# skywoodsz/qm_control

Hardware: NVIDIA H100
Metric: mpc_wbc_iters_per_s (higher is better)
Workload: dtype f64

## Files before the change

### qm_control_b200/csrc/capi.cu

```cuda
#include <cuda_runtime.h>

#include <algorithm>
#include <cmath>
#include <cstdio>
#include <cstring>
#include <string>
#include <vector>

#include "../../include/qmb200.h"
#include "host/qm_config.h"
#include "kernels/mpc_api.cuh"
#include "kernels/ctrl_api.cuh"
#include "kernels/sim_api.cuh"
#include "kernels/payload_est_api.cuh"
#include "kernels/state_est_api.cuh"
#include "kernels/attitude_api.cuh"
#include "kernels/slip_api.cuh"
#include "kernels/gait_api.cuh"

namespace qmb {
void launch_wbc_update(const DevModel* mdl, int B, const double* x_des, const double* u_des, const double* rbd, const int32_t* mode, const double* period, const double* time,
                       double* input_last, int variant, double* cmd, int32_t* status, cudaStream_t stream, int b0 = 0, int b1 = -1, int32_t* diag = nullptr,
                       const double* srbd = nullptr, const double* payload = nullptr);
int wbc_configure_device();
int mpc_configure_device();
}

using namespace qmb;

static thread_local std::string g_create_error;

struct RobotArray {
  int width; std::vector<double> host; double* d = nullptr;
  const double* dev() const { return host.empty() ? nullptr : d; }
};

struct qmb200_handle {
  HostModel hm;
  DevModel* d_model = nullptr;
  int B = 0, nmax = 0, variant = 0, device = 0;
  cudaStream_t stream = nullptr;
  std::string err, task_file, reference_file;
  int64_t launches = 0;
  double *d_xdes = nullptr, *d_udes = nullptr, *d_input_last = nullptr;
  int32_t *d_mode = nullptr, *d_wbc_diag = nullptr, *d_safety = nullptr;
  char* stage = nullptr; size_t stage_bytes = 0;
  MpcBuffers mpc;
  std::vector<void*> allocs;
  bool profiling = false; cudaEvent_t ev[8] = {nullptr};
  double kernel_ms[7] = {0, 0, 0, 0, 0, 0, 0}; int64_t kernel_calls = 0; bool ev_pending = false;
  static constexpr int MAX_CHUNKS = 8;
  TargetParams target_prm{}; ControlLawParams law_prm{0, 0.0, 0.5};
  double hw_delay = 0.0; double *hw_ring_cmd = nullptr, *hw_ring_stamp = nullptr; int32_t* hw_ring_state = nullptr;
  void* comm = nullptr; int comm_ranks = 0, comm_rank = 0; double* d_send = nullptr;
  SimParams sim_prm{};
  RobotArray mu{1}, payload{8};
  RobotArray terrain{3};
  struct { std::vector<double> host; double* d = nullptr; int n_tiles = 0, nx = 0, ny = 0; double cell = 0.0; } tiles;
  RobotArray mpayload{8}, srbd{SRBD_DBL};
  qmb200_payload_est_params est_prm{}; double* d_est = nullptr;
  qmb200_sensor_params sensor_prm{};
  qmb200_state_est_params se_prm{}; double* d_se = nullptr;
  RobotArray se_ground{3};
  qmb200_attitude_params at_prm{}; double* d_at = nullptr;
  qmb200_slip_params sl_prm{}; double* d_sl = nullptr;
  struct {
    std::vector<GsTemplate> table; GsTemplate* d_table = nullptr; GsRobot* d_robots = nullptr; int32_t* d_cursor = nullptr;
    double* d_t = nullptr; int32_t* d_tmpl = nullptr; double* d_vel = nullptr; int n_cmd = 0; double stance_time = 0.0;
    int32_t* d_ee_kind = nullptr; double* d_ee = nullptr;
  } gs;
  bool model_on_device = false;
  int chunks = 1; cudaStream_t cs[MAX_CHUNKS] = {nullptr}; cudaEvent_t fork_ev = nullptr, join_ev[MAX_CHUNKS] = {nullptr};
};

namespace {
template <class T> bool dalloc(qmb200_handle* h, T** p, size_t count) {
  void* q = nullptr; cudaError_t e = cudaMalloc(&q, count * sizeof(T));
  if (e != cudaSuccess) { h->err = std::string("cudaMalloc failed: ") + cudaGetErrorString(e); return false; }
  cudaMemsetAsync(q, 0, count * sizeof(T), h->stream); h->allocs.push_back(q); *p = static_cast<T*>(q); return true;
}
SimParams default_sim_params();
qmb200_payload_est_params default_est_params();
qmb200_state_est_params default_state_est_params(const DevModel& d);
qmb200_attitude_params default_attitude_params();
qmb200_slip_params default_slip_params();
int fail(qmb200_handle* h, const std::string& msg) { if (h) h->err = msg; else g_create_error = msg; return -1; }
#define QMB_CUDA(h, call) do { cudaError_t e_ = (call); if (e_ != cudaSuccess) return fail(h, std::string(#call) + ": " + cudaGetErrorString(e_)); } while (0)

HostModel config_model(const qmb200_config* cfg) {
  HostModel hm = build_host_model(cfg->task_file, cfg->urdf_file, cfg->reference_file, cfg->wbc_gains_file ? cfg->wbc_gains_file : "");
  if (cfg->time_horizon > 0) hm.dev.time_horizon = cfg->time_horizon;
  if (cfg->dt > 0) hm.dev.dt = cfg->dt;
  return hm;
}
int push_model(qmb200_handle* h) {
  QMB_CUDA(h, cudaMemcpyAsync(h->d_model, &h->hm.dev, sizeof(DevModel), cudaMemcpyHostToDevice, h->stream)); QMB_CUDA(h, cudaStreamSynchronize(h->stream)); return 0;
}

struct RobotRows { RobotArray* a; const double* rows; };
int set_robot_arrays(qmb200_handle* h, std::initializer_list<RobotRows> sets) {
  const size_t B = (size_t)h->B;
  QMB_CUDA(h, cudaSetDevice(h->device));
  for (const RobotRows& s : sets) if (s.rows && !s.a->d && !dalloc(h, &s.a->d, B * s.a->width)) return -4;
  QMB_CUDA(h, cudaDeviceSynchronize());
  for (const RobotRows& s : sets) if (s.rows) QMB_CUDA(h, cudaMemcpy(s.a->d, s.rows, B * s.a->width * 8, cudaMemcpyHostToDevice));
  for (const RobotRows& s : sets) { if (s.rows) s.a->host.assign(s.rows, s.rows + B * s.a->width); else s.a->host.clear(); }
  return 0;
}

class Staging {
 public:
  static constexpr size_t ROBOT_BYTES = 243 * 8, ALIGN = 256, STAGE_SLICES = 10;
  explicit Staging(qmb200_handle* h) : h_(h) {}
  int open() {
    QMB_CUDA(h_, cudaSetDevice(h_->device));
    if (!h_->stage) {
      const size_t bytes = (size_t)h_->B * ROBOT_BYTES + STAGE_SLICES * ALIGN;
      if (!dalloc(h_, &h_->stage, bytes)) return -4;
      h_->stage_bytes = bytes;
    }
    return 0;
  }
  template <class T> const T* in(const T* src, size_t n) {
    if (!src) return nullptr;
    T* d = slice<T>(n); note(cudaMemcpyAsync(d, src, n * sizeof(T), cudaMemcpyHostToDevice, h_->stream)); return d;
  }
  template <class T> T* inout(T* p, size_t n) { T* d = const_cast<T*>(in<T>(p, n)); back_.push_back({p, d, n * sizeof(T)}); return d; }
  template <class T> T* out(T* p, size_t n) { T* d = slice<T>(n); back_.push_back({p, d, n * sizeof(T)}); return d; }
  int done(int rc) {
    if (rc) return rc;
    for (const Back& b : back_) note(cudaMemcpyAsync(b.host, b.dev, b.bytes, cudaMemcpyDeviceToHost, h_->stream));
    note(cudaStreamSynchronize(h_->stream));
    return err_.empty() ? 0 : fail(h_, err_);
  }

 private:
  struct Back { void* host; const void* dev; size_t bytes; };
  qmb200_handle* h_; size_t used_ = 0; std::vector<Back> back_; std::string err_;
  void note(cudaError_t e) { if (e != cudaSuccess && err_.empty()) err_ = std::string("staging copy: ") + cudaGetErrorString(e); }
  template <class T> T* slice(size_t n) {
    const size_t at = used_, bytes = n * sizeof(T);
    if (at + bytes > h_->stage_bytes) { if (err_.empty()) err_ = "staging arena too small"; return reinterpret_cast<T*>(h_->stage); }
    used_ = (at + bytes + ALIGN - 1) / ALIGN * ALIGN; return reinterpret_cast<T*>(h_->stage + at);
  }
};

void wbc_launch(qmb200_handle* h, const double* x_des, const double* u_des, const double* rbd, const int32_t* mode, const double* period, const double* time, double* cmd,
                int32_t* status, cudaStream_t s, int b0 = 0, int b1 = -1) {
  launch_wbc_update(h->d_model, h->B, x_des, u_des, rbd, mode, period, time, h->d_input_last, h->variant, cmd, status, s, b0, b1, h->d_wbc_diag, h->srbd.dev(), h->mpayload.dev());
  h->launches += 1;
}
}

extern "C" {

int qmb200_create(const qmb200_config* cfg, qmb200_handle** out) {
  if (!cfg || !out) return fail(nullptr, "qmb200_create: null argument");
  if (!cfg->task_file || !cfg->urdf_file || !cfg->reference_file) return fail(nullptr, "qmb200_create: task/urdf/reference file required");
  if (cfg->batch < 1) return fail(nullptr, "qmb200_create: batch must be >= 1");
  qmb200_handle* h = new qmb200_handle();
  try {
    h->hm = config_model(cfg);
    InfoFile ref(cfg->reference_file), task(cfg->task_file);
    h->target_prm.com_height = ref.number("comHeight"); h->target_prm.target_displacement_velocity = ref.number("targetDisplacementVelocity");
    h->target_prm.target_rotation_velocity = ref.number("targetRotationVelocity"); h->target_prm.time_to_target = task.number("mpc.timeHorizon");
    for (int j = 0; j < NJ; ++j) h->target_prm.default_joint_state[j] = h->hm.default_joint_state[j];
  } catch (const std::exception& e) { g_create_error = e.what(); delete h; return -2; }
  h->task_file = cfg->task_file; h->reference_file = cfg->reference_file;
  h->sim_prm = default_sim_params(); h->est_prm = default_est_params(); h->se_prm = default_state_est_params(h->hm.dev); h->at_prm = default_attitude_params();
  h->sl_prm = default_slip_params();
  h->B = cfg->batch; h->variant = cfg->wbc_variant; h->device = cfg->device; h->law_prm.variant = cfg->wbc_variant == QMB200_WBC_HIERARCHICAL_MPC ? 1 : 0;
  const int nint = (int)std::ceil(h->hm.dev.time_horizon / h->hm.dev.dt - 1e-9);
  h->nmax = cfg->max_nodes > 0 ? cfg->max_nodes : nint + 1 + 20;
  int ndev = 0; cudaError_t e = cudaGetDeviceCount(&ndev);
  if (e != cudaSuccess || ndev == 0) { g_create_error = std::string("qmb200_create: no CUDA device (") + cudaGetErrorString(e) + ") — this library has no CPU fallback"; delete h; return -3; }
  if (cudaSetDevice(cfg->device) != cudaSuccess) { g_create_error = "qmb200_create: cudaSetDevice failed"; delete h; return -3; }
  cudaStreamCreateWithFlags(&h->stream, cudaStreamNonBlocking);
  if (wbc_configure_device() != 0 || mpc_configure_device() != 0) { g_create_error = std::string("qmb200_create: cudaFuncSetAttribute failed: ") + cudaGetErrorString(cudaGetLastError()); qmb200_destroy(h); return -3; }
  const size_t B = (size_t)h->B;
  bool ok = dalloc(h, &h->d_model, 1) && dalloc(h, &h->d_xdes, B * NX) && dalloc(h, &h->d_udes, B * NU) && dalloc(h, &h->d_input_last, B * NU) && dalloc(h, &h->d_mode, B) &&
            dalloc(h, &h->d_wbc_diag, B) && dalloc(h, &h->d_safety, B) && dalloc(h, &h->d_send, B * NJ);
  if (ok) { std::string merr; ok = mpc_alloc(h->mpc, h->B, h->nmax, merr, h->allocs, h->stream); if (!ok) h->err = merr; }
  if (!ok) { g_create_error = h->err; qmb200_destroy(h); return -4; }
  if (push_model(h)) { g_create_error = "qmb200_create: " + h->err; qmb200_destroy(h); return -4; }
  *out = h; return 0;
}

void qmb200_destroy(qmb200_handle* h) {
  if (!h) return;
  cudaSetDevice(h->device);
  qmb200_comm_destroy(h);
  if (h->stream) { cudaStreamSynchronize(h->stream); cudaStreamDestroy(h->stream); }
  for (int c = 0; c < qmb200_handle::MAX_CHUNKS; ++c) { if (h->cs[c]) { cudaStreamSynchronize(h->cs[c]); cudaStreamDestroy(h->cs[c]); } if (h->join_ev[c]) cudaEventDestroy(h->join_ev[c]); }
  if (h->fork_ev) cudaEventDestroy(h->fork_ev);
  for (void* p : h->allocs) cudaFree(p);
  if (h->tiles.d) cudaFree(h->tiles.d);
  if (h->d_est) cudaFree(h->d_est);
  if (h->d_se) cudaFree(h->d_se);
  if (h->d_at) cudaFree(h->d_at);
  if (h->d_sl) cudaFree(h->d_sl);
  cudaFree(h->gs.d_table); cudaFree(h->gs.d_robots); cudaFree(h->gs.d_cursor); cudaFree(h->gs.d_t); cudaFree(h->gs.d_tmpl); cudaFree(h->gs.d_vel);
  cudaFree(h->gs.d_ee_kind); cudaFree(h->gs.d_ee);
  delete h;
}

const char* qmb200_last_error(const qmb200_handle* h) { return h ? h->err.c_str() : g_create_error.c_str(); }

int64_t qmb200_debug_model_blob(const qmb200_config* cfg, void* out, int64_t capacity) {
  if (!cfg || !cfg->task_file || !cfg->urdf_file || !cfg->reference_file) { g_create_error = "qmb200_debug_model_blob: task/urdf/reference file required"; return -1; }
  try {
    const HostModel hm = config_model(cfg);
    if (out && capacity >= (int64_t)sizeof(DevModel)) std::memcpy(out, &hm.dev, sizeof(DevModel));
    return (int64_t)sizeof(DevModel);
  } catch (const std::exception& e) { g_create_error = e.what(); return -2; }
}

static_assert(SRBD_DBL == QMB200_SRBD, "per-robot SRBD block of include/qmb200.h");
static_assert(RBD_EE_QUAT + 4 == QMB200_RBD, "rbd layout of include/qmb200.h");
}
namespace {
std::string payload_error(const double* payload, size_t n, const char* who) {
  for (size_t b = 0; b < n; ++b) {
    const double* p = payload + 8 * b;
    for (int i = 0; i < 8; ++i) if (!std::isfinite(p[i])) return std::string(who) + ": payload must be finite";
    if (p[0] < 0.0 || p[4] < 0.0) return std::string(who) + ": payload masses must be >= 0";
  }
  return "";
}
int model_rows_sync(const qmb200_handle* hc) {
  qmb200_handle* h = const_cast<qmb200_handle*>(hc);
  if (!h->model_on_device) return 0;
  const size_t B = (size_t)h->B;
  QMB_CUDA(h, cudaSetDevice(h->device)); QMB_CUDA(h, cudaDeviceSynchronize());
  QMB_CUDA(h, cudaMemcpy(h->mpayload.host.data(), h->mpayload.d, B * 8 * 8, cudaMemcpyDeviceToHost));
// ... 116 lines not shown
```

### qm_control_b200/csrc/kernels/dev_common.cuh

```cuda
#pragma once
#include <cuda_runtime.h>
#include <math.h>
#include <stddef.h>
#include <stdint.h>

#ifdef __CUDACC__
#define QMB_HD __host__ __device__ __forceinline__
#else
#define QMB_HD inline
#endif

namespace qmb {

constexpr int NQ = 24;
constexpr int NJ = 18;
constexpr int NB = 19;
constexpr int NX = 30;
constexpr int NU = 30;
constexpr int NDEC = 36;
constexpr unsigned FULL = 0xffffffffu;
constexpr int RBD_ZYX = 0, RBD_POS = 3, RBD_JPOS = 6, RBD_W = 24, RBD_V = 27, RBD_JVEL = 30, RBD_EE_POS = 48, RBD_EE_QUAT = 51;

struct DevModel {
  int parent[NJ];
// ... 40 lines not shown
QMB_HD const SrbdConst* srbd_of(const DevModel* mdl, const double* srbd, int b) {
  return srbd ? reinterpret_cast<const SrbdConst*>(srbd + (size_t)SRBD_DBL * b) : reinterpret_cast<const SrbdConst*>(&mdl->total_mass);
}

#ifdef __CUDACC__
__device__ __forceinline__ double warp_sum(double v) {
#pragma unroll
  for (int o = 16; o > 0; o >>= 1) v += __shfl_xor_sync(FULL, v, o);
  return v;
}
__device__ __forceinline__ double warp_max(double v) {
#pragma unroll
  for (int o = 16; o > 0; o >>= 1) v = fmax(v, __shfl_xor_sync(FULL, v, o));
  return v;
}
__device__ __forceinline__ double warp_min(double v) {
#pragma unroll
  for (int o = 16; o > 0; o >>= 1) v = fmin(v, __shfl_xor_sync(FULL, v, o));
  return v;
}
__device__ __forceinline__ void warp_argmax(double& v, int& idx) {
#pragma unroll
  for (int o = 16; o > 0; o >>= 1) {
    double ov = __shfl_xor_sync(FULL, v, o); int oi = __shfl_xor_sync(FULL, idx, o);
    if (ov > v || (ov == v && oi < idx)) { v = ov; idx = oi; }
  }
}
__device__ __forceinline__ void warp_argmax_nonneg(double& v, int& idx, bool active) {
  const unsigned long long b = active ? (unsigned long long)__double_as_longlong(v) : 0ull;
  const unsigned hi = (unsigned)(b >> 32), lo = (unsigned)b;
  const unsigned mh = __reduce_max_sync(FULL, hi);
  const unsigned ml = __reduce_max_sync(FULL, hi == mh ? lo : 0u);
  const unsigned m = __ballot_sync(FULL, active && hi == mh && lo == ml);
  if (m == 0u) { v = -1.0; idx = 0; return; }
  idx = __ffs(m) - 1; v = __longlong_as_double((long long)(((unsigned long long)mh << 32) | ml));
}
__device__ __forceinline__ void warp_argmin(double& v, int& idx) {
#pragma unroll
  for (int o = 16; o > 0; o >>= 1) {
    double ov = __shfl_xor_sync(FULL, v, o); int oi = __shfl_xor_sync(FULL, idx, o);
    if (ov < v || (ov == v && oi < idx)) { v = ov; idx = oi; }
  }
}

#endif

QMB_HD void cross3(const double* a, const double* b, double* c) {
  c[0] = a[1] * b[2] - a[2] * b[1]; c[1] = a[2] * b[0] - a[0] * b[2]; c[2] = a[0] * b[1] - a[1] * b[0];
}
QMB_HD void cross3_add(const double* a, const double* b, double* c) {
  c[0] += a[1] * b[2] - a[2] * b[1]; c[1] += a[2] * b[0] - a[0] * b[2]; c[2] += a[0] * b[1] - a[1] * b[0];
}
QMB_HD double dot3(const double* a, const double* b) { return a[0] * b[0] + a[1] * b[1] + a[2] * b[2]; }
QMB_HD void matvec3(const double* M, const double* v, double* o) {
  o[0] = M[0] * v[0] + M[1] * v[1] + M[2] * v[2]; o[1] = M[3] * v[0] + M[4] * v[1] + M[5] * v[2]; o[2] = M[6] * v[0] + M[7] * v[1] + M[8] * v[2];
}
QMB_HD void matTvec3(const double* M, const double* v, double* o) {
  o[0] = M[0] * v[0] + M[3] * v[1] + M[6] * v[2]; o[1] = M[1] * v[0] + M[4] * v[1] + M[7] * v[2]; o[2] = M[2] * v[0] + M[5] * v[1] + M[8] * v[2];
}
QMB_HD void matmul3(const double* A, const double* B, double* C) {
#pragma unroll
  for (int i = 0; i < 3; ++i)
#pragma unroll
    for (int j = 0; j < 3; ++j) C[3 * i + j] = A[3 * i] * B[j] + A[3 * i + 1] * B[3 + j] + A[3 * i + 2] * B[6 + j];
}
QMB_HD void matmul3_nt(const double* A, const double* B, double* C) {
#pragma unroll
  for (int i = 0; i < 3; ++i)
#pragma unroll
    for (int j = 0; j < 3; ++j) C[3 * i + j] = A[3 * i] * B[3 * j] + A[3 * i + 1] * B[3 * j + 1] + A[3 * i + 2] * B[3 * j + 2];
}
QMB_HD void rot_zyx(double z, double y, double x, double* R) {
  double sz, cz, sy, cy, sx, cx; sincos(z, &sz, &cz); sincos(y, &sy, &cy); sincos(x, &sx, &cx);
  R[0] = cz * cy; R[1] = cz * sy * sx - sz * cx; R[2] = cz * sy * cx + sz * sx;
  R[3] = sz * cy; R[4] = sz * sy * sx + cz * cx; R[5] = sz * sy * cx - cz * sx;
  R[6] = -sy;     R[7] = cy * sx;                R[8] = cy * cx;
}
QMB_HD void euler_rate_map(double z, double y, double* T) {
  double sz, cz, sy, cy; sincos(z, &sz, &cz); sincos(y, &sy, &cy);
  T[0] = 0; T[1] = -sz; T[2] = cy * cz; T[3] = 0; T[4] = cz; T[5] = cy * sz; T[6] = 1; T[7] = 0; T[8] = -sy;
}
QMB_HD void euler_rate_map_dot_times(double z, double y, const double* ed, double* o) {
  double sz, cz, sy, cy; sincos(z, &sz, &cz); sincos(y, &sy, &cy);
  const double zd = ed[0], yd = ed[1];
  o[0] = (-cz * zd) * ed[1] + (-sy * yd * cz - cy * sz * zd) * ed[2];
  o[1] = (-sz * zd) * ed[1] + (-sy * yd * sz + cy * cz * zd) * ed[2];
  o[2] = (-cy * yd) * ed[2];
}
QMB_HD void rot_zyx_sc(const double* tr, double* R) {
  const double sz = tr[0], cz = tr[1], sy = tr[2], cy = tr[3], sx = tr[4], cx = tr[5];
  R[0] = cz * cy; R[1] = cz * sy * sx - sz * cx; R[2] = cz * sy * cx + sz * sx;
  R[3] = sz * cy; R[4] = sz * sy * sx + cz * cx; R[5] = sz * sy * cx - cz * sx;
  R[6] = -sy;     R[7] = cy * sx;                R[8] = cy * cx;
}
QMB_HD void euler_rate_map_sc(const double* tr, double* T) {
  const double sz = tr[0], cz = tr[1], sy = tr[2], cy = tr[3];
  T[0] = 0; T[1] = -sz; T[2] = cy * cz; T[3] = 0; T[4] = cz; T[5] = cy * sz; T[6] = 1; T[7] = 0; T[8] = -sy;
}
QMB_HD void euler_rate_map_dot_times_sc(const double* tr, const double* ed, double* o) {
  const double sz = tr[0], cz = tr[1], sy = tr[2], cy = tr[3]; const double zd = ed[0], yd = ed[1];
  o[0] = (-cz * zd) * ed[1] + (-sy * yd * cz - cy * sz * zd) * ed[2];
  o[1] = (-sz * zd) * ed[1] + (-sy * yd * sz + cy * cz * zd) * ed[2];
  o[2] = (-cy * yd) * ed[2];
}
QMB_HD void rot_to_quat_xyzw(const double* m, double* o) {
  const double t = m[0] + m[4] + m[8];
// ... 78 lines not shown
```

### qm_control_b200/csrc/kernels/wbc_kernel.cu

```cuda
#include "dev_common.cuh"
#include "payload.cuh"
#include "wlinalg.cuh"

namespace qmb {

constexpr int LDM = 25;
constexpr int LDZ = 37;
constexpr int LZ = 19;
constexpr int MAXR = 24;
constexpr int LJC = 9;
constexpr int MAXW = 20;
#ifndef QMB_WBC_WARPS
#define QMB_WBC_WARPS 8
#endif
constexpr int WBC_WARPS = QMB_WBC_WARPS;

enum { ST_OK = 0, ST_ITER_CAP = 1, ST_TOO_MANY_ROWS = 2, ST_NAN = 4 };

struct EeWs { double Jee[6 * LDM], djv_ee[6], ee_m_pos[3], ee_m_vel[3], ee_m_rot[9], ee_m_w[3], ee_d_pos[3], ee_d_vel[3], ee_d_rot[9]; };
struct QpWs {
  union ZA { struct Q { double Z[36 * LZ];
                        double AR[MAXR * LDZ];
                      } q;
             RbdWs rbd;
             __device__ ZA() {} } za;
  union AH { double Ah[MAXR * LZ];
             EeWs ee; __device__ AH() {} } ah;
  double G[18 * 19 / 2 + 1];
  double tau[MAXR], tauc[MAXW];
  double xbar[36], dx[36], g[36], y[36], s[36], zac[LZ + 1], rhs[MAXR], bp[MAXR], bh[MAXR], lam[MAXW], t18[MAXR];
  int perm[MAXR], permc[MAXW], wset[MAXW];
};
static_assert(LZ * MAXR + LZ * MAXW <= MAXR * LDZ, "W1 and Wc share the row build area");
static_assert(sizeof(RbdWs) <= sizeof(double) * (36 * LZ + MAXR * LDZ), "rigid-body workspace overlays Z + AR only");

struct WbcSmem {
  double q[NQ], v[NQ], qd[NQ], vd[NQ];
  double M[NQ * LDM], nle[NQ];
  double Jc[12 * LJC], djv_f[12], fpos_m[12], fvel_m[12], fpos_d[12], fvel_d[12];
  double Tm[9], wdot_base[3], base_acc[6], fdes[12], lim[NJ], vstar[56];
  QpWs qp;
};

struct IneqCtx { const WbcSmem* sm; int mode; int nc; double mu; int lfp, ffp; };
__device__ __forceinline__ int foot_first(int ffp, int f) { return (ffp >> (4 * f)) & 15; }
__device__ __forceinline__ double jt_force(const WbcSmem* sm, int lfp, int jn, const double* F) {
  if (jn >= 12) return 0.0;
  const int lg = jn / 3, f = (lfp >> (2 * lg)) & 3, d = jn - 3 * lg; const double* J = sm->Jc + 3 * f * LJC + 6 + d;
  return J[0] * F[3 * f] + J[LJC] * F[3 * f + 1] + J[2 * LJC] * F[3 * f + 2];
}

__device__ __forceinline__ int stance_foot_by_rank(int mode, int rank) { int k = 0; for (int f = 0; f < 4; ++f) if (contact_flag(mode, f)) { if (k == rank) return f; ++k; } return -1; }

__device__ __forceinline__ double ineq_row_dot(const IneqCtx& c, int i, const double* x) {
  if (i < 36) {
    const int jn = i < 18 ? i : i - 18; const double* Mr = c.sm->M + (6 + jn) * LDM; double s = 0.0;
    for (int k = 0; k < NQ; ++k) s += Mr[k] * x[k];
    s -= jt_force(c.sm, c.lfp, jn, x + NQ);
    return i < 18 ? s : -s;
  }
  const int r = i - 36; const int foot = stance_foot_by_rank(c.mode, r / 5); const int t = r % 5; const double* F = x + NQ + 3 * foot;
  if (t == 0) return -F[2];
  if (t == 1) return F[0] - c.mu * F[2];
  if (t == 2) return -F[0] - c.mu * F[2];
  if (t == 3) return F[1] - c.mu * F[2];
  return -F[1] - c.mu * F[2];
}
__device__ __forceinline__ double ineq_rhs(const IneqCtx& c, int i) {
  double f = 0.0;
  if (i < 18) f = c.sm->lim[i] - c.sm->nle[6 + i]; else if (i < 36) f = c.sm->lim[i - 18] + c.sm->nle[6 + i - 18];
  return f + c.sm->vstar[i];
}
__device__ __forceinline__ double ineq_row_elem(const IneqCtx& c, int i, int k) {
  if (i < 36) { const int jn = i < 18 ? i : i - 18; const double sgn = i < 18 ? 1.0 : -1.0; if (k < NQ) return sgn * c.sm->M[(6 + jn) * LDM + k];
    const int r = k - NQ, d = jn - foot_first(c.ffp, r / 3); return (d >= 0 && d < 3) ? -sgn * c.sm->Jc[r * LJC + 6 + d] : 0.0; }
  const int r = i - 36; const int foot = stance_foot_by_rank(c.mode, r / 5); const int t = r % 5; const int kk = k - NQ - 3 * foot;
  if (kk < 0 || kk > 2) return 0.0;
  if (kk == 2) return t == 0 ? -1.0 : -c.mu;
  if (kk == 0) return t == 1 ? 1.0 : (t == 2 ? -1.0 : 0.0);
  return t == 3 ? 1.0 : (t == 4 ? -1.0 : 0.0);
}

__device__ int cod_lstsq(QpWs& qp, double* W, int n, int r, int ldw, const double* rhs, double* y, double* G, int lane) {
  const int k = w_qrcp(W, n, r, ldw, qp.tau, qp.perm, 1e-11, lane);
  for (int i = lane; i < n; i += 32) y[i] = 0.0;
  __syncwarp();
  if (k == 0) return 0;
  if (k == r) {
    for (int c = 0; c < k; ++c) {
      double part = 0.0; if (lane < c) part = W[lane + c * ldw] * y[lane];
      const double s = warp_sum(part);
      if (lane == 0) y[c] = (rhs[qp.perm[c]] - s) / W[c + c * ldw];
      __syncwarp();
    }
  } else {
    { int a = 0, b = lane; while (b > a) { b -= a + 1; ++a; }
      while (a < k) { double s = 0.0; for (int c = a; c < r; ++c) s += W[a + c * ldw] * W[b + c * ldw]; G[tri(a) + b] = s;
        b += 32; while (b > a) { b -= a + 1; ++a; } } }
    if (lane < k) { double s = 0.0; for (int c = lane; c < r; ++c) s += W[lane + c * ldw] * rhs[qp.perm[c]]; qp.t18[lane] = s; }
    __syncwarp();
    w_cholesky(G, k, lane);
    w_chol_solve(G, k, qp.t18, lane);
    if (lane < k) y[lane] = qp.t18[lane];
    __syncwarp();
  }
  w_apply_q(W, n, k, ldw, qp.tau, y, lane);
  return k;
}

__device__ int build_level(WbcSmem& sm, const DevModel* __restrict__ mdl, int level, int mode, int variant, bool init_phase, int ffp, int lane) {
  QpWs& qp = sm.qp; double* Ap = qp.za.q.AR; const EeWs& ee = qp.ah.ee; int nc = 0; for (int f = 0; f < 4; ++f) nc += contact_flag(mode, f);
  int rows = 0;
  if (level == 0) rows = 18;
  else if (level == 1) rows = (variant == 0) ? (init_phase ? 6 : 10 + 3 * (4 - nc)) : (6 + 3 * (4 - nc));
  else rows = (variant == 0) ? 14 : 12;
  for (int e = lane; e < rows * LDZ; e += 32) Ap[e] = 0.0;
  __syncwarp();
  if (level == 0) {
    for (int e = lane; e < 6 * 36; e += 32) { const int r = e / 36, k = e % 36; Ap[r * LDZ + k] = (k < NQ) ? sm.M[r * LDM + k] : -sm.Jc[(k - NQ) * LJC + r]; }
    if (lane < 6) qp.bp[lane] = -sm.nle[lane];
    int row = 6;
    for (int f = 0; f < 4; ++f) if (contact_flag(mode, f)) { if (lane < 27) { const int a = lane / 9, c = lane - 9 * a; Ap[(row + a) * LDZ + (c < 6 ? c : foot_first(ffp, f) + c)] = sm.Jc[(3 * f + a) * LJC + c]; } if (lane < 3) qp.bp[row + lane] = -sm.djv_f[3 * f + lane]; row += 3; }
    for (int f = 0; f < 4; ++f) if (!contact_flag(mode, f)) { if (lane < 3) { Ap[(row + lane) * LDZ + NQ + 3 * f + lane] = 1.0; qp.bp[row + lane] = 0.0; } row += 3; }
  } else if (level == 1) {
    int row = 0;
    if (variant == 0 && init_phase) {
      if (lane < 6) { const int k = NQ - 6 + lane; Ap[lane * LDZ + k] = 1.0; qp.bp[lane] = mdl->arm_joint_kp[lane] * (sm.qd[k] - sm.q[k]) + mdl->arm_joint_kd[lane] * (sm.vd[k] - sm.v[k]); }
      row = 6;
    } else {
      if (lane == 0) { Ap[2] = 1.0; qp.bp[0] = sm.base_acc[2] + mdl->base_height_kp * (sm.qd[2] - sm.q[2]) + mdl->base_height_kd * (sm.vd[2] - sm.v[2]); }
      if (lane < 3) {
        const int r = lane; for (int k = 0; k < 3; ++k) Ap[(1 + r) * LDZ + 3 + k] = sm.Tm[3 * r + k];
        double wM[3], wD[3]; matvec3(sm.Tm, sm.v + 3, wM); matvec3(sm.Tm, sm.vd + 3, wD);
        double Rm[9], Rr[9], err[3]; rot_zyx(sm.q[3], sm.q[4], sm.q[5], Rm); rot_zyx(sm.qd[3], sm.qd[4], sm.qd[5], Rr); rotation_error_world(Rr, Rm, err);
        double tdd[3], tde[3]; matvec3(sm.Tm, sm.base_acc + 3, tdd); euler_rate_map_dot_times(sm.q[3], sm.q[4], sm.vd + 3, tde);
        qp.bp[1 + r] = tdd[r] + tde[r] + mdl->base_angular_kp * err[r] + mdl->base_angular_kd * (wD[r] - wM[r]) - sm.wdot_base[r];
      }
      row = 4;
      if (variant == 0) {
        for (int e = lane; e < 6 * NQ; e += 32) { const int a = e / NQ, k = e % NQ; const bool zero = (a >= 3 && k >= 3 && k < 6); Ap[(row + a) * LDZ + k] = zero ? 0.0 : ee.Jee[a * LDM + k]; }
        if (lane < 3) qp.bp[row + lane] = mdl->ee_linear_kp[lane] * (ee.ee_d_pos[lane] - ee.ee_m_pos[lane]) + mdl->ee_linear_kd[lane] * (ee.ee_d_vel[lane] - ee.ee_m_vel[lane]) - ee.djv_ee[lane];
        if (lane == 3) { double err[3]; rotation_error_world(ee.ee_d_rot, ee.ee_m_rot, err);
          for (int a = 0; a < 3; ++a) qp.bp[row + 3 + a] = mdl->ee_angular_kp[a] * err[a] - mdl->ee_angular_kd[a] * ee.ee_m_w[a] - (ee.djv_ee[3 + a] - sm.wdot_base[a]); }
        row += 6;
      } else {
        if (lane < 2) { Ap[(row + lane) * LDZ + lane] = 1.0; qp.bp[row + lane] = sm.base_acc[lane] + mdl->base_linear_kp * (sm.qd[lane] - sm.q[lane]) + mdl->base_linear_kd * (sm.vd[lane] - sm.v[lane]); }
        row += 2;
      }
      for (int f = 0; f < 4; ++f) if (!contact_flag(mode, f)) {
        if (lane < 27) { const int a = lane / 9, c = lane - 9 * a; Ap[(row + a) * LDZ + (c < 6 ? c : foot_first(ffp, f) + c)] = 100.0 * sm.Jc[(3 * f + a) * LJC + c]; }
        if (lane < 3) { const int i = 3 * f + lane; qp.bp[row + lane] = 100.0 * (mdl->kp_swing * (sm.fpos_d[i] - sm.fpos_m[i]) + mdl->kd_swing * (sm.fvel_d[i] - sm.fvel_m[i]) - sm.djv_f[i]); }
        row += 3;
      }
    }
  } else {
    if (lane < 12) { Ap[lane * LDZ + NQ + lane] = 1.0; qp.bp[lane] = sm.fdes[lane]; }
    if (variant == 0 && lane < 2) { Ap[(12 + lane) * LDZ + lane] = 1.0; qp.bp[12 + lane] = sm.base_acc[lane] + mdl->base_linear_kp * (sm.qd[lane] - sm.q[lane]) + mdl->base_linear_kd * (sm.vd[lane] - sm.v[lane]); }
  }
  __syncwarp();
  return rows;
}

__device__ __forceinline__ void project_task(QpWs& qp, int rows, int off, int nz, int lane) {
  const double* Ap = qp.za.q.AR; const double* Z = qp.za.q.Z;
  for (int e = lane; e < rows * nz; e += 32) { const int i = e / nz, c = e - i * nz; const double* a = Ap + i * LDZ; double s0 = 0.0, s1 = 0.0;
#pragma unroll 6
    for (int k = 0; k < 36; k += 2) { s0 = fma(a[k], Z[k * LZ + off + c], s0); s1 = fma(a[k + 1], Z[(k + 1) * LZ + off + c], s1); }
    qp.ah.Ah[i * LZ + c] = s0 + s1; }
  if (lane < rows) { const double* a = Ap + lane * LDZ; double s = 0.0; for (int k = 0; k < 36; ++k) s = fma(a[k], qp.xbar[k], s); qp.bh[lane] = qp.bp[lane] - s; }
  __syncwarp();
}

__device__ int solve_level(WbcSmem& sm, const IneqCtx& ic, int rows, int off, int nzc, int& nw, int lane, int& iters_out, int iter_cap) {
  QpWs& qp = sm.qp; const int nz = nzc - off; const int nineq = 36 + 5 * ic.nc; int status = 0;
  if (nz <= 0) return 0;
  const double* Z = qp.za.q.Z; const double* Ah = qp.ah.Ah; double* W1 = qp.za.q.AR; double* Wc = qp.za.q.AR + LZ * MAXR;
  if (lane < LZ + 1) qp.zac[lane] = 0.0;
  __syncwarp();
  bool converged = false;
  for (int iter = 0; iter < iter_cap; ++iter) {
    iters_out = iter + 1;
    int kc = 0;
    if (nw > 0) {
      for (int k = 0; k < nw; ++k) {
        const int wi = qp.wset[k]; qp.y[lane] = ineq_row_elem(ic, wi, lane); if (lane < 4) qp.y[32 + lane] = ineq_row_elem(ic, wi, 32 + lane);
        __syncwarp();
        if (lane < nz) { double s0 = 0.0, s1 = 0.0;
#pragma unroll 6
          for (int j = 0; j < 36; j += 2) { s0 = fma(qp.y[j], Z[j * LZ + off + lane], s0); s1 = fma(qp.y[j + 1], Z[(j + 1) * LZ + off + lane], s1); }
// ... 7 lines not shown
      }
    }
    for (int e = lane; e < rows * LZ; e += 32) W1[e] = Ah[e];
    if (lane < rows) { const double* a = Ah + lane * LZ; double s = 0.0; for (int c = 0; c < nz; ++c) s = fma(a[c], qp.zac[c], s); qp.rhs[lane] = qp.bh[lane] - s; }
    __syncwarp();
    if (kc > 0) w_apply_qt_cols(Wc, nz, kc, LZ, qp.tauc, W1, rows, LZ, lane);
    const int nfree = nz - kc;
    for (int i = lane; i < nz; i += 32) qp.s[i] = 0.0;
    __syncwarp();
    if (nfree > 0) cod_lstsq(qp, W1 + kc, nfree, rows, LZ, qp.rhs, qp.s + kc, qp.G, lane);
    if (kc > 0) w_apply_q(Wc, nz, kc, LZ, qp.tauc, qp.s, lane);
    for (int i = lane; i < 36; i += 32) { double d = 0.0; for (int c = 0; c < nz; ++c) d = fma(Z[i * LZ + off + c], qp.s[c], d); qp.dx[i] = d; }
    __syncwarp();
    double dmax = 0.0, xmax = 0.0; for (int i = lane; i < 36; i += 32) { dmax = fmax(dmax, fabs(qp.dx[i])); xmax = fmax(xmax, fabs(qp.xbar[i])); }
    dmax = warp_max(dmax); xmax = warp_max(xmax);
    bool full_step = true;
    if (dmax > 1e-12 * (1.0 + xmax)) {
      double alpha = 1.0; int blk = -1;
      for (int i = lane; i < nineq; i += 32) {
        bool inw = false; for (int k = 0; k < nw; ++k) inw |= (qp.wset[k] == i);
        if (inw) continue;
        const double ad = ineq_row_dot(ic, i, qp.dx);
        if (ad > 1e-12 * (1.0 + dmax)) { double r = (ineq_rhs(ic, i) - ineq_row_dot(ic, i, qp.xbar)) / ad; if (r < 0.0) r = 0.0; if (r < alpha) { alpha = r; blk = i; } }
      }
      { double a = alpha; int b = (blk < 0) ? 0x7fffffff : blk; warp_argmin(a, b); alpha = a; blk = (alpha < 1.0) ? b : -1; }
      for (int i = lane; i < 36; i += 32) qp.xbar[i] += alpha * qp.dx[i];
      if (lane < nz) qp.zac[lane] += alpha * qp.s[lane];
      __syncwarp();
      if (blk >= 0) { if (nw >= MAXW) { status |= ST_TOO_MANY_ROWS; break; } if (lane == 0) qp.wset[nw] = blk; nw += 1; __syncwarp(); full_step = false; }
    }
    if (!full_step) continue;
    if (nw == 0) { converged = true; break; }
    if (lane < rows) { const double* a = Ah + lane * LZ; double s = 0.0; for (int c = 0; c < nz; ++c) s = fma(a[c], qp.zac[c], s); qp.rhs[lane] = s - qp.bh[lane]; }
    __syncwarp();
    for (int c = lane; c < nz; c += 32) { double s = 0.0; for (int r = 0; r < rows; ++r) s = fma(Ah[r * LZ + c], qp.rhs[r], s); qp.g[c] = s; }
    __syncwarp();
    w_apply_qt(Wc, nz, kc, LZ, qp.tauc, qp.g, lane);
    double gmax = 0.0; for (int i = lane; i < nz; i += 32) gmax = fmax(gmax, fabs(qp.g[i])); gmax = warp_max(gmax);
    for (int c = kc - 1; c >= 0; --c) {
      double part = 0.0; if (lane > c && lane < kc) part = Wc[c + lane * LZ] * qp.lam[lane];
      const double s = warp_sum(part);
      if (lane == 0) qp.lam[c] = (-qp.g[c] - s) / Wc[c + c * LZ];
      __syncwarp();
    }
    double lmin = (lane < kc) ? qp.lam[lane] : 1e300; int li = lane; warp_argmin(lmin, li);
    if (lmin >= -1e-9 * (1.0 + gmax)) { converged = true; break; }
    { const int drop = qp.permc[li]; int keep = -1; if (lane < nw) { int src = lane < drop ? lane : lane + 1; keep = (src < nw) ? qp.wset[src] : -1; } __syncwarp(); if (lane < nw - 1) qp.wset[lane] = keep;
      nw -= 1; __syncwarp(); }
  }
  if (!converged) status |= ST_ITER_CAP;
  return status;
}

__global__ void __launch_bounds__(32 * WBC_WARPS) wbc_update_kernel(const DevModel* __restrict__ mdl, int b0, int B, const double* __restrict__ x_des, const double* __restrict__ u_des,
                                                                   const double* __restrict__ rbd_meas, const int32_t* __restrict__ mode_in, const double* __restrict__ period_in,
                                                                   const double* __restrict__ time_in, double* __restrict__ input_last, int variant,
                                                                   double* __restrict__ cmd_out, int32_t* __restrict__ status_out, int32_t* __restrict__ diag_out,
                                                                   const double* __restrict__ srbd, const double* __restrict__ payload) {
  extern __shared__ __align__(16) unsigned char smem_raw[];
  const int warp = threadIdx.x >> 5, lane = threadIdx.x & 31;
  const int b = b0 + blockIdx.x * (int)(blockDim.x >> 5) + warp;
  if (b >= B) return;
  WbcSmem& sm = reinterpret_cast<WbcSmem*>(smem_raw)[warp];
  const int mode = mode_in[b]; const double period = period_in[b]; const double time = time_in[b];
  int nc = 0; for (int f = 0; f < 4; ++f) nc += contact_flag(mode, f);

  const double* xdes = x_des + (size_t)b * NX; const double* udes = u_des + (size_t)b * NU;
  if (lane < 12) sm.fdes[lane] = udes[lane];
  const int lfp = mdl->leg_foot[0] | (mdl->leg_foot[1] << 2) | (mdl->leg_foot[2] << 4) | (mdl->leg_foot[3] << 6);
  const int ffp = mdl->foot_leg[0] | (mdl->foot_leg[1] << 4) | (mdl->foot_leg[2] << 8) | (mdl->foot_leg[3] << 12);
  if (lane < NJ) sm.lim[lane] = (lane < 12) ? mdl->effort[lane % 3] : mdl->effort[lane];
  for (int i = lane; i < 56; i += 32) sm.vstar[i] = 0.0;
  rbd_read(rbd_meas + (size_t)b * 55, sm.q, sm.v, sm.Tm, lane);
  if (lane < NQ) sm.qd[lane] = xdes[6 + lane];
  __syncwarp();

  RbdWs* ws = &sm.qp.za.rbd; EeWs& ee = sm.qp.ah.ee;
  rbd_kinematics<true>(mdl, sm.q, sm.v, ws, lane);
  rbd_inertias(mdl, ws, lane, 1);
  if (payload) { if (lane < 2) payload_load(mdl, ws, lane, payload + (size_t)b * 8 + 4 * lane, true); __syncwarp(); }
  rbd_accumulate(mdl, ws, lane, true);
  rbd_mass_matrix_nle(mdl, ws, sm.M, LDM, sm.nle, lane);
  for (int f = 0; f < 4; ++f) {
    const int body = mdl->foot_body[f]; double pw[3]; foot_point(mdl, ws, f, pw);
    if (lane < 9) { const double* S = ws->S[lane < 6 ? lane : foot_first(ffp, f) + lane]; double col[3]; point_vel(S, pw, col);
      for (int a = 0; a < 3; ++a) sm.Jc[(3 * f + a) * LJC + lane] = col[a]; }
    if (lane == 0) { double vel[3], acc[3]; point_vel_acc(ws->V[body], ws->A[body], pw, vel, acc); for (int a = 0; a < 3; ++a) { sm.fpos_m[3 * f + a] = pw[a]; sm.fvel_m[3 * f + a] = vel[a]; sm.djv_f[3 * f + a] = acc[a]; } }
  }
  {
    const int body = mdl->ee_body; double pw[3]; ee_pose(mdl, ws, pw, lane == 0 ? ee.ee_m_rot : nullptr);
    point_jacobian(ws, pw, 12, 17, ee.Jee, LDM, lane);
    if (lane < NQ) { const bool on = (lane < 6) || (lane >= 18); for (int a = 0; a < 3; ++a) ee.Jee[(3 + a) * LDM + lane] = on ? ws->S[lane][a] : 0.0; }
    if (lane == 0) { double vel[3], acc[3]; point_vel_acc(ws->V[body], ws->A[body], pw, vel, acc); for (int a = 0; a < 3; ++a) { ee.ee_m_pos[a] = pw[a]; ee.ee_m_vel[a] = vel[a]; ee.djv_ee[a] = acc[a]; ee.djv_ee[3 + a] = ws->A[body][a]; ee.ee_m_w[a] = ws->V[body][a]; sm.wdot_base[a] = ws->A[0][a]; } }
  }
  __syncwarp();

  double jacc = 0.0;
  if (lane < NJ) { const double uj = udes[12 + lane]; jacc = (uj - input_last[(size_t)b * NU + 12 + lane]) / period; sm.vd[6 + lane] = uj; }
  __syncwarp();
  if (lane < NU) input_last[(size_t)b * NU + lane] = udes[lane];
  double A22inv[9], A12[9];
  if (lane == 0) {
    const SrbdConst* sc = srbd_of(mdl, srbd, b);
    double R[9], T[9]; rot_zyx(sm.qd[3], sm.qd[4], sm.qd[5], R); euler_rate_map(sm.qd[3], sm.qd[4], T);
    double c[3]; matvec3(R, sc->c_nom, c);
    double RI[9], RIRt[9], A22[9]; matmul3(R, sc->I_nom, RI); matmul3_nt(RI, R, RIRt); matmul3(RIRt, T, A22); inv3(A22, A22inv);
    const double Sx[9] = {0, -c[2], c[1], c[2], 0, -c[0], -c[1], c[0], 0}; double ST[9]; matmul3(Sx, T, ST); for (int i = 0; i < 9; ++i) A12[i] = sc->m * ST[i];
    double ha[3] = {sc->m * xdes[3], sc->m * xdes[4], sc->m * xdes[5]}, ed[3]; matvec3(A22inv, ha, ed);
    double t[3]; matvec3(A12, ed, t);
    for (int a = 0; a < 3; ++a) { sm.vd[a] = xdes[a] - t[a] / sc->m; sm.vd[3 + a] = ed[a]; }
  }
  __syncwarp();
  rbd_kinematics<true>(mdl, sm.qd, sm.vd, ws, lane);
  rbd_inertias(mdl, ws, lane, 2);
  if (payload) { if (lane < 2) payload_load(mdl, ws, lane, payload + (size_t)b * 8 + 4 * lane, false); __syncwarp(); }
  rbd_accumulate(mdl, ws, lane, true);
  double Phi[6] = {0, 0, 0, 0, 0, 0};
  if (lane < NJ) { inertia_apply(ws->Ic[lane + 1], ws->S[6 + lane], Phi); for (int i = 0; i < 6; ++i) Phi[i] *= jacc; }
  for (int i = 0; i < 6; ++i) Phi[i] = warp_sum(Phi[i]);
  for (int f = 0; f < 4; ++f) {
    double pw[3]; foot_point(mdl, ws, f, pw);
    if (lane == 0) { double vel[3]; point_vel(ws->V[mdl->foot_body[f]], pw, vel); for (int a = 0; a < 3; ++a) { sm.fpos_d[3 * f + a] = pw[a]; sm.fvel_d[3 * f + a] = vel[a]; } }
  }
  if (lane == 0) {
    double pw[3], vel[3]; ee_pose(mdl, ws, pw, ee.ee_d_rot); point_vel(ws->V[mdl->ee_body], pw, vel);
    for (int a = 0; a < 3; ++a) { ee.ee_d_pos[a] = pw[a]; ee.ee_d_vel[a] = vel[a]; }
    const SrbdConst* sc = srbd_of(mdl, srbd, b);
    const double mt = ws->Ic[0][0]; const double com[3] = {ws->Ic[0][1] / mt, ws->Ic[0][2] / mt, ws->Ic[0][3] / mt};
    double lin[3] = {0, 0, -9.81 * sc->m}, ang[3] = {0, 0, 0};
    for (int f = 0; f < 4; ++f) { const double* F = sm.fdes + 3 * f; const double r[3] = {sm.fpos_d[3 * f] - com[0], sm.fpos_d[3 * f + 1] - com[1], sm.fpos_d[3 * f + 2] - com[2]}; lin[0] += F[0]; lin[1] += F[1]; lin[2] += F[2]; cross3_add(r, F, ang); }
    const double* Fb = ws->F[0]; double cf[3]; cross3(com, Fb + 3, cf);
    double cp[3]; cross3(com, Phi + 3, cp);
    for (int a = 0; a < 3; ++a) { lin[a] -= Fb[3 + a] + Phi[3 + a]; ang[a] -= (Fb[a] - cf[a]) + (Phi[a] - cp[a]); }
    double ed[3]; matvec3(A22inv, ang, ed); double t[3]; matvec3(A12, ed, t);
    for (int a = 0; a < 3; ++a) { sm.base_acc[a] = (lin[a] - t[a]) / sc->m; sm.base_acc[3 + a] = ed[a]; }
  }
  __syncwarp();

  QpWs& qp = sm.qp; IneqCtx ic{&sm, mode, nc, mdl->wbc_friction, lfp, ffp}; int status = 0;
  const bool init_phase = time < 10.0;
  double* AR = qp.za.q.AR; double* Z = qp.za.q.Z;
  for (int i = lane; i < 36; i += 32) qp.xbar[i] = 0.0;
  __syncwarp();
  const int nineq = 36 + 5 * nc; const int cap0 = mdl->wbc_iter_cap0, cap = mdl->wbc_iter_cap; int it0 = 0;
  unsigned vmask0 = 0, vmask1 = 0;
  int k0 = 0;
  for (int it = 0; it < cap0; ++it) {
    int r = build_level(sm, mdl, 0, mode, variant, init_phase, ffp, lane); it0 = it + 1;
    for (int i = 0; i < nineq; ++i) { const bool in = (i < 32) ? ((vmask0 >> i) & 1u) : ((vmask1 >> (i - 32)) & 1u); if (in) { if (r >= MAXR) { status |= ST_TOO_MANY_ROWS; break; }
        for (int k = lane; k < 36; k += 32) AR[r * LDZ + k] = ineq_row_elem(ic, i, k); if (lane == 0) qp.bp[r] = ineq_rhs(ic, i); ++r; } }
    __syncwarp();
    k0 = cod_lstsq(qp, AR, 36, r, LDZ, qp.bp, qp.xbar, Z, lane);
    __syncwarp();
    unsigned n0 = 0, n1 = 0;
    for (int i = lane; i < nineq; i += 32) { const double val = ineq_row_dot(ic, i, qp.xbar) - ineq_rhs(ic, i); const double sc = 1e-9 * (1.0 + fabs(ineq_rhs(ic, i)));
      const bool inV = (i < 32) ? ((vmask0 >> i) & 1u) : ((vmask1 >> (i - 32)) & 1u);
      if (val > sc || (inV && val >= -sc)) { if (i < 32) n0 |= 1u << i; else n1 |= 1u << (i - 32); } }
    for (int o = 16; o > 0; o >>= 1) { n0 |= __shfl_xor_sync(FULL, n0, o); n1 |= __shfl_xor_sync(FULL, n1, o); }
    if (n0 == vmask0 && n1 == vmask1) break;
    vmask0 = n0; vmask1 = n1;
    if (it == cap0 - 1) status |= ST_ITER_CAP;
  }
  for (int i = lane; i < nineq; i += 32) { const double val = ineq_row_dot(ic, i, qp.xbar) - ineq_rhs(ic, i); sm.vstar[i] = val > 0.0 ? val : 0.0; }
  __syncwarp();
  int off = 0, nzc = 0, nw = 0, it1 = 0, it2 = 0;
  {
    if (vmask0 | vmask1) {
      const int rows0 = build_level(sm, mdl, 0, mode, variant, init_phase, ffp, lane);
      k0 = w_qrcp(AR, 36, rows0, LDZ, qp.tau, qp.perm, 1e-11, lane);
    }
    nzc = 36 - k0;
    if (nzc > LZ - 1) { status |= ST_TOO_MANY_ROWS; nzc = 0; }
    else w_form_q_tail(AR, 36, k0, LDZ, qp.tau, Z, LZ, lane);
  }
  for (int level = 1; level <= 2 && nzc > 0; ++level) {
    const int rows = build_level(sm, mdl, level, mode, variant, init_phase, ffp, lane);
    const int nz = nzc - off;
    if (nz <= 0) break;
    project_task(qp, rows, off, nz, lane);
    status |= solve_level(sm, ic, rows, off, nzc, nw, lane, level == 1 ? it1 : it2, cap);
    if (level == 1) {
      const int k = w_qrcp(qp.ah.Ah, nz, rows, LZ, qp.tau, qp.perm, 1e-11, lane);
      w_apply_q_right(qp.ah.Ah, nz, k, LZ, qp.tau, Z, 36, LZ, off, lane);
      off += k;
    }
  }
  double* out = cmd_out + (size_t)b * 54;
  for (int i = lane; i < 36; i += 32) out[i] = qp.xbar[i];
  bool bad = false;
  if (lane < NJ) { const double* Mr = sm.M + (6 + lane) * LDM; double s = sm.nle[6 + lane]; for (int k = 0; k < NQ; ++k) s += Mr[k] * qp.xbar[k]; s -= jt_force(&sm, lfp, lane, qp.xbar + NQ); out[36 + lane] = s; bad = !isfinite(s); }
  if (__any_sync(FULL, bad)) status |= ST_NAN;
  if (lane == 0) { status_out[b] = status; if (diag_out) diag_out[b] = (it0 & 0xff) | ((it1 & 0xff) << 8) | ((it2 & 0xff) << 16) | ((nw & 0xff) << 24); }
}

static_assert(sizeof(WbcSmem) * WBC_WARPS <= 227 * 1024, "WBC shared-memory budget exceeded");
size_t wbc_smem_bytes() { return sizeof(WbcSmem) * WBC_WARPS; }

void launch_wbc_update(const DevModel* mdl, int B, const double* x_des, const double* u_des, const double* rbd, const int32_t* mode, const double* period, const double* time,
                       double* input_last, int variant, double* cmd, int32_t* status, cudaStream_t stream, int b0, int b1, int32_t* diag, const double* srbd, const double* payload) {
  if (b1 < 0) b1 = B; if (b1 <= b0) return;
  const int nb = b1 - b0; const int wpc = WBC_WARPS;
  const int grid = (nb + wpc - 1) / wpc;
  wbc_update_kernel<<<grid, 32 * wpc, sizeof(WbcSmem) * wpc, stream>>>(mdl, b0, b1, x_des, u_des, rbd, mode, period, time, input_last, variant, cmd, status, diag, srbd, payload);
}

int wbc_configure_device() { return (int)cudaFuncSetAttribute(wbc_update_kernel, cudaFuncAttributeMaxDynamicSharedMemorySize, (int)wbc_smem_bytes()); }

}
```

Before: 24.40.

## Reorder WBC robots by previous solver iteration counts to balance warps

Adds a single-block counting-sort kernel that orders the robots by the sum of QP iteration counts recorded in last call's diagnostics, so the WBC kernel assigns work in descending expected cost. This aims to reduce load imbalance and tail latency across blocks. It also adds a min-blocks-per-SM launch bound, unrolls the Phi warp reduction, and rewrites small indexing into select form so arrays stay in registers. The cost is an extra kernel launch per update, and the ordering relies on iteration counts staying similar between calls.

```diff
diff --git a/qm_control_b200/csrc/capi.cu b/qm_control_b200/csrc/capi.cu
--- a/qm_control_b200/csrc/capi.cu
+++ b/qm_control_b200/csrc/capi.cu
@@ -21,7 +21,8 @@
 namespace qmb {
 void launch_wbc_update(const DevModel* mdl, int B, const double* x_des, const double* u_des, const double* rbd, const int32_t* mode, const double* period, const double* time,
                        double* input_last, int variant, double* cmd, int32_t* status, cudaStream_t stream, int b0 = 0, int b1 = -1, int32_t* diag = nullptr,
-                       const double* srbd = nullptr, const double* payload = nullptr);
+                       const double* srbd = nullptr, const double* payload = nullptr,
+                       int32_t* order = nullptr);
 int wbc_configure_device();
 int mpc_configure_device();
 }
@@ -44,6 +45,7 @@
   int64_t launches = 0;
   double *d_xdes = nullptr, *d_udes = nullptr, *d_input_last = nullptr;
   int32_t *d_mode = nullptr, *d_wbc_diag = nullptr, *d_safety = nullptr;
+  int32_t* d_wbc_order = nullptr;
   char* stage = nullptr; size_t stage_bytes = 0;
   MpcBuffers mpc;
   std::vector<void*> allocs;
@@ -147,7 +149,7 @@
 
 void wbc_launch(qmb200_handle* h, const double* x_des, const double* u_des, const double* rbd, const int32_t* mode, const double* period, const double* time, double* cmd,
                 int32_t* status, cudaStream_t s, int b0 = 0, int b1 = -1) {
-  launch_wbc_update(h->d_model, h->B, x_des, u_des, rbd, mode, period, time, h->d_input_last, h->variant, cmd, status, s, b0, b1, h->d_wbc_diag, h->srbd.dev(), h->mpayload.dev());
+  launch_wbc_update(h->d_model, h->B, x_des, u_des, rbd, mode, period, time, h->d_input_last, h->variant, cmd, status, s, b0, b1, h->d_wbc_diag, h->srbd.dev(), h->mpayload.dev(), h->d_wbc_order);
   h->launches += 1;
 }
 }
@@ -179,7 +181,7 @@
   if (wbc_configure_device() != 0 || mpc_configure_device() != 0) { g_create_error = std::string("qmb200_create: cudaFuncSetAttribute failed: ") + cudaGetErrorString(cudaGetLastError()); qmb200_destroy(h); return -3; }
   const size_t B = (size_t)h->B;
   bool ok = dalloc(h, &h->d_model, 1) && dalloc(h, &h->d_xdes, B * NX) && dalloc(h, &h->d_udes, B * NU) && dalloc(h, &h->d_input_last, B * NU) && dalloc(h, &h->d_mode, B) &&
-            dalloc(h, &h->d_wbc_diag, B) && dalloc(h, &h->d_safety, B) && dalloc(h, &h->d_send, B * NJ);
+            dalloc(h, &h->d_wbc_diag, B) && dalloc(h, &h->d_wbc_order, B) && dalloc(h, &h->d_safety, B) && dalloc(h, &h->d_send, B * NJ);
   if (ok) { std::string merr; ok = mpc_alloc(h->mpc, h->B, h->nmax, merr, h->allocs, h->stream); if (!ok) h->err = merr; }
   if (!ok) { g_create_error = h->err; qmb200_destroy(h); return -4; }
   if (push_model(h)) { g_create_error = "qmb200_create: " + h->err; qmb200_destroy(h); return -4; }
diff --git a/qm_control_b200/csrc/kernels/dev_common.cuh b/qm_control_b200/csrc/kernels/dev_common.cuh
--- a/qm_control_b200/csrc/kernels/dev_common.cuh
+++ b/qm_control_b200/csrc/kernels/dev_common.cuh
@@ -116,6 +116,7 @@
   c[0] += a[1] * b[2] - a[2] * b[1]; c[1] += a[2] * b[0] - a[0] * b[2]; c[2] += a[0] * b[1] - a[1] * b[0];
 }
 QMB_HD double dot3(const double* a, const double* b) { return a[0] * b[0] + a[1] * b[1] + a[2] * b[2]; }
+QMB_HD double sel3(const double* a, int i) { return i == 0 ? a[0] : (i == 1 ? a[1] : a[2]); }
 QMB_HD void matvec3(const double* M, const double* v, double* o) {
   o[0] = M[0] * v[0] + M[1] * v[1] + M[2] * v[2]; o[1] = M[3] * v[0] + M[4] * v[1] + M[5] * v[2]; o[2] = M[6] * v[0] + M[7] * v[1] + M[8] * v[2];
 }
diff --git a/qm_control_b200/csrc/kernels/wbc_kernel.cu b/qm_control_b200/csrc/kernels/wbc_kernel.cu
--- a/qm_control_b200/csrc/kernels/wbc_kernel.cu
+++ b/qm_control_b200/csrc/kernels/wbc_kernel.cu
@@ -41,6 +41,7 @@
   double Tm[9], wdot_base[3], base_acc[6], fdes[12], lim[NJ], vstar[56];
   QpWs qp;
 };
+constexpr int WBC_CTAS_PER_SM = (int)((228 * 1024) / (sizeof(WbcSmem) * WBC_WARPS + 1024));
 
 struct IneqCtx { const WbcSmem* sm; int mode; int nc; double mu; int lfp, ffp; };
 __device__ __forceinline__ int foot_first(int ffp, int f) { return (ffp >> (4 * f)) & 15; }
@@ -134,7 +135,7 @@
         double wM[3], wD[3]; matvec3(sm.Tm, sm.v + 3, wM); matvec3(sm.Tm, sm.vd + 3, wD);
         double Rm[9], Rr[9], err[3]; rot_zyx(sm.q[3], sm.q[4], sm.q[5], Rm); rot_zyx(sm.qd[3], sm.qd[4], sm.qd[5], Rr); rotation_error_world(Rr, Rm, err);
         double tdd[3], tde[3]; matvec3(sm.Tm, sm.base_acc + 3, tdd); euler_rate_map_dot_times(sm.q[3], sm.q[4], sm.vd + 3, tde);
-        qp.bp[1 + r] = tdd[r] + tde[r] + mdl->base_angular_kp * err[r] + mdl->base_angular_kd * (wD[r] - wM[r]) - sm.wdot_base[r];
+        qp.bp[1 + r] = sel3(tdd, r) + sel3(tde, r) + mdl->base_angular_kp * sel3(err, r) + mdl->base_angular_kd * (sel3(wD, r) - sel3(wM, r)) - sm.wdot_base[r];
       }
       row = 4;
       if (variant == 0) {
@@ -248,15 +249,16 @@
   return status;
 }
 
-__global__ void __launch_bounds__(32 * WBC_WARPS) wbc_update_kernel(const DevModel* __restrict__ mdl, int b0, int B, const double* __restrict__ x_des, const double* __restrict__ u_des,
+__global__ void __launch_bounds__(32 * WBC_WARPS, WBC_CTAS_PER_SM) wbc_update_kernel(const DevModel* __restrict__ mdl, int b0, int B, const double* __restrict__ x_des, const double* __restrict__ u_des,
                                                                    const double* __restrict__ rbd_meas, const int32_t* __restrict__ mode_in, const double* __restrict__ period_in,
                                                                    const double* __restrict__ time_in, double* __restrict__ input_last, int variant,
                                                                    double* __restrict__ cmd_out, int32_t* __restrict__ status_out, int32_t* __restrict__ diag_out,
-                                                                   const double* __restrict__ srbd, const double* __restrict__ payload) {
+                                                                   const double* __restrict__ srbd, const double* __restrict__ payload, const int32_t* __restrict__ order) {
   extern __shared__ __align__(16) unsigned char smem_raw[];
   const int warp = threadIdx.x >> 5, lane = threadIdx.x & 31;
-  const int b = b0 + blockIdx.x * (int)(blockDim.x >> 5) + warp;
-  if (b >= B) return;
+  const int slot = b0 + blockIdx.x * (int)(blockDim.x >> 5) + warp;
+  if (slot >= B) return;
+  const int b = order ? order[slot] : slot;
   WbcSmem& sm = reinterpret_cast<WbcSmem*>(smem_raw)[warp];
   const int mode = mode_in[b]; const double period = period_in[b]; const double time = time_in[b];
   int nc = 0; for (int f = 0; f < 4; ++f) nc += contact_flag(mode, f);
@@ -313,6 +315,7 @@
   rbd_accumulate(mdl, ws, lane, true);
   double Phi[6] = {0, 0, 0, 0, 0, 0};
   if (lane < NJ) { inertia_apply(ws->Ic[lane + 1], ws->S[6 + lane], Phi); for (int i = 0; i < 6; ++i) Phi[i] *= jacc; }
+#pragma unroll
   for (int i = 0; i < 6; ++i) Phi[i] = warp_sum(Phi[i]);
   for (int f = 0; f < 4; ++f) {
     double pw[3]; foot_point(mdl, ws, f, pw);
@@ -374,7 +377,8 @@
     const int nz = nzc - off;
     if (nz <= 0) break;
     project_task(qp, rows, off, nz, lane);
-    status |= solve_level(sm, ic, rows, off, nzc, nw, lane, level == 1 ? it1 : it2, cap);
+    int its = 0; status |= solve_level(sm, ic, rows, off, nzc, nw, lane, its, cap);
+    if (level == 1) it1 = its; else it2 = its;
     if (level == 1) {
       const int k = w_qrcp(qp.ah.Ah, nz, rows, LZ, qp.tau, qp.perm, 1e-11, lane);
       w_apply_q_right(qp.ah.Ah, nz, k, LZ, qp.tau, Z, 36, LZ, off, lane);
@@ -389,15 +393,30 @@
   if (lane == 0) { status_out[b] = status; if (diag_out) diag_out[b] = (it0 & 0xff) | ((it1 & 0xff) << 8) | ((it2 & 0xff) << 16) | ((nw & 0xff) << 24); }
 }
 
+constexpr int WBC_ORDER_KEYS = 64;
+__device__ __forceinline__ int wbc_order_key(int32_t d) { return min((d & 0xff) + ((d >> 8) & 0xff) + ((d >> 16) & 0xff), WBC_ORDER_KEYS - 1); }
+__global__ void __launch_bounds__(1024) wbc_order_kernel(int b0, int b1, const int32_t* __restrict__ diag, int32_t* __restrict__ order) {
+  __shared__ int start[WBC_ORDER_KEYS];
+  if (threadIdx.x < WBC_ORDER_KEYS) start[threadIdx.x] = 0;
+  __syncthreads();
+  for (int b = b0 + threadIdx.x; b < b1; b += blockDim.x) atomicAdd(&start[wbc_order_key(diag[b])], 1);
+  __syncthreads();
+  if (threadIdx.x == 0) { int s = b0; for (int k = WBC_ORDER_KEYS - 1; k >= 0; --k) { const int c = start[k]; start[k] = s; s += c; } }
+  __syncthreads();
+  for (int b = b0 + threadIdx.x; b < b1; b += blockDim.x) order[atomicAdd(&start[wbc_order_key(diag[b])], 1)] = b;
+}
+
 static_assert(sizeof(WbcSmem) * WBC_WARPS <= 227 * 1024, "WBC shared-memory budget exceeded");
 size_t wbc_smem_bytes() { return sizeof(WbcSmem) * WBC_WARPS; }
 
 void launch_wbc_update(const DevModel* mdl, int B, const double* x_des, const double* u_des, const double* rbd, const int32_t* mode, const double* period, const double* time,
-                       double* input_last, int variant, double* cmd, int32_t* status, cudaStream_t stream, int b0, int b1, int32_t* diag, const double* srbd, const double* payload) {
+                       double* input_last, int variant, double* cmd, int32_t* status, cudaStream_t stream, int b0, int b1, int32_t* diag, const double* srbd, const double* payload,
+                       int32_t* order) {
   if (b1 < 0) b1 = B; if (b1 <= b0) return;
+  if (diag && order) wbc_order_kernel<<<1, 1024, 0, stream>>>(b0, b1, diag, order); else order = nullptr;
   const int nb = b1 - b0; const int wpc = WBC_WARPS;
   const int grid = (nb + wpc - 1) / wpc;
-  wbc_update_kernel<<<grid, 32 * wpc, sizeof(WbcSmem) * wpc, stream>>>(mdl, b0, b1, x_des, u_des, rbd, mode, period, time, input_last, variant, cmd, status, diag, srbd, payload);
+  wbc_update_kernel<<<grid, 32 * wpc, sizeof(WbcSmem) * wpc, stream>>>(mdl, b0, b1, x_des, u_des, rbd, mode, period, time, input_last, variant, cmd, status, diag, srbd, payload, order);
 }
 
 int wbc_configure_device() { return (int)cudaFuncSetAttribute(wbc_update_kernel, cudaFuncAttributeMaxDynamicSharedMemorySize, (int)wbc_smem_bytes()); }
```

Result: no change. 24.65 (median of 6 runs) (+1.0%).
